# xenji/kafka-topic-analyzer

Measured on AMD Instinct MI355X. Metric: records/sec whole-node + achieved HBM GB/s, 256-part 256B-mean synthetic topic, higher is better.
Workload: dtype u64; 1 GPU; c4: 256-partition synthetic topic, mixed key/value sizes (mean record ~256 B), partitions sharded p % n_gpus; records_per_gpu=1073741824, partitions=256, partition_order=random, bytes_per_record=20, parallelism=partition-sharded x1, forced_collectives=False, exchange=none (1 GPU)

## Files before the change

kafka_topic_analyzer_amd/csrc/kta_api.hip:

```cpp
#include "../../include/kta_hip.h"
#include "kta_compact_delete.h"
#include "kta_compaction.h"
#include "kta_internal.h"
#include "kta_kernels.h"
#include "kta_murmur2.h"
#include "kta_payload.h"
#include "kta_record_batches.h"
#include "kta_segments.h"
#include "kta_size_bins.h"

#include <limits.h>
#include <math.h>
#include <stdio.h>
#include <string.h>

#include <algorithm>
#include <new>
#include <cstdlib>
#include <string>
#include <time.h>
#include <vector>

namespace {

// ... 191 lines not shown

kta_batch *find_allocation(kta_ctx *ctx, const int32_t *p, int32_t *kta_batch::*col, uint64_t *rec0)
{
    const uintptr_t a = reinterpret_cast<uintptr_t>(p);
    for (kta_batch &e : ctx->compact_batches) {
        const uintptr_t lo = reinterpret_cast<uintptr_t>(e.*col);
        if (!p || a < lo || a >= lo + allocation_rows(e) * 4) continue;
        *rec0 = (a - lo) / 4;
        return &e;
    }
    return nullptr;
}

kta_internal_columns columns_at(const kta_internal_columns &rb, uint64_t at)
{
    kta_internal_columns r = rb;
    r.rec0 += at;
    if (!rb.hdr) r.partition += at, r.key_len += at, r.val_len += at, r.ts_ms += at;
    return r;
}
kta::ScanColumns scan_columns(const kta_internal_columns &rb, uint64_t at)
{
    const kta_internal_columns r = columns_at(rb, at);
    return kta::ScanColumns{r.partition, r.key_len, r.val_len, r.ts_ms, r.hdr, r.rec0, r.sum, r.mark};
}
kta::SketchColumns sketch_columns(const kta_internal_columns &rb, const kta_batch *c, uint64_t at)
{
    const kta_internal_columns r = columns_at(rb, at);
    return kta::SketchColumns{r.partition, r.hdr, r.rec0, c->key_len + at, c->key_off + at, c->key_bytes};
}

bool aligned16(const void *p) { return (reinterpret_cast<uintptr_t>(p) & 15u) == 0; }

int widen_lens_for_keys(kta_ctx *ctx, const kta_batch *c, uint64_t n)
{
    uint64_t rec0 = 0;
    const kta_batch *e = find_allocation(ctx, c->key_len, &kta_batch::key_len, &rec0);
    if (!e || e->key_bytes) return KTA_OK;
    const uint64_t rows = allocation_rows(*e), hi = rec0 + n < rows ? rec0 + n : rows;
    KTA_HIP(ctx, kta::launch_tiles_to_raw(e->partition, e->ts_ms, e->key_len, e->val_len, e->tile_hdr, rec0, hi, 2u, true, ctx->s_compute));
    return KTA_OK;
}

constexpr uint64_t kAliveUniqueNum = 2, kAliveUniqueDen = 5;
constexpr int kAliveBackoff = 7;

kta::WrittenList written_list(kta_ctx *ctx) { return kta::WrittenList{ctx->d_written.get(), ctx->d_written_n.get(), ctx->d_written.size()}; }
// ... 1132 lines not shown
    if (!h->partition || !h->key_len || !h->val_len || !h->ts_ms || !d->partition || !d->key_len || !d->val_len || !d->ts_ms)
        return fail(ctx, KTA_ERR_INVALID, "metric columns missing");
    KTA_HIP(ctx, hipSetDevice(ctx->device));
    kta_internal_columns r{};
    int rc = kta_internal_resolve(ctx, d, &r);
    if (rc != KTA_OK) return rc;
    KTA_HIP(ctx, hipStreamSynchronize(ctx->s_compute));
    if (!r.hdr || !r.keyless) {
        KTA_HIP(ctx, hipMemcpy(d->key_len, h->key_len, n * 4, hipMemcpyHostToDevice));
        KTA_HIP(ctx, hipMemcpy(d->val_len, h->val_len, n * 4, hipMemcpyHostToDevice));
    }
    if (!r.hdr) {
        KTA_HIP(ctx, hipMemcpy(d->partition, h->partition, n * 4, hipMemcpyHostToDevice));
        KTA_HIP(ctx, hipMemcpy(d->ts_ms, h->ts_ms, n * 8, hipMemcpyHostToDevice));
        return KTA_OK;
    }
    if (r.rec0 % KTA_TILE_RECORDS)
        return fail(ctx, KTA_ERR_INVALID, "a tile-compact batch is written from a tile boundary");
    const uint64_t nt = tiles_of(n);
    std::vector<int32_t> part(nt * KTA_TILE_RECORDS, 0);
    std::vector<int64_t> ts(nt * KTA_TILE_RECORDS, 0);
    std::vector<kta_tile_hdr> hdr(nt);
    std::vector<kta_tile_sum> sum(nt);
    std::vector<uint32_t> mark(nt, 0u);
    std::vector<int32_t> klen, vlen;
    if (r.keyless) {
        klen.assign(nt * KTA_TILE_RECORDS, 0);
        vlen.assign(nt * KTA_TILE_RECORDS, 0);
    }
    for (uint64_t T = 0; T < nt; T++) {
        const uint64_t a = T * KTA_TILE_RECORDS, m = n - a < KTA_TILE_RECORDS ? n - a : KTA_TILE_RECORDS;
        hdr[T] = kta::tile_pack_host(h->partition + a, h->ts_ms + a, h->key_len + a, h->val_len + a, m, r.keyless, part.data() + a, ts.data() + a,
                                     r.keyless ? klen.data() + a : nullptr, r.keyless ? vlen.data() + a : nullptr, &sum[T]);
        if (r.mark) mark[T] = kta::tile_plane_host(hdr[T], h->partition + a, h->key_len + a, h->val_len + a, m, ts.data() + a);
    }
    if (r.keyless) {
        KTA_HIP(ctx, hipMemcpy(r.key_len + r.rec0, klen.data(), klen.size() * 4, hipMemcpyHostToDevice));
        KTA_HIP(ctx, hipMemcpy(r.val_len + r.rec0, vlen.data(), vlen.size() * 4, hipMemcpyHostToDevice));
    }
    KTA_HIP(ctx, hipMemcpy(r.partition + r.rec0, part.data(), part.size() * 4, hipMemcpyHostToDevice));
    KTA_HIP(ctx, hipMemcpy(r.ts_ms + r.rec0, ts.data(), ts.size() * 8, hipMemcpyHostToDevice));
    KTA_HIP(ctx, hipMemcpy(r.hdr + r.rec0 / KTA_TILE_RECORDS, hdr.data(), nt * sizeof(kta_tile_hdr), hipMemcpyHostToDevice));
    if (r.sum) KTA_HIP(ctx, hipMemcpy(r.sum + r.rec0 / KTA_TILE_RECORDS, sum.data(), nt * sizeof(kta_tile_sum), hipMemcpyHostToDevice));
    if (r.mark) KTA_HIP(ctx, hipMemcpy(r.mark + r.rec0 / KTA_TILE_RECORDS, mark.data(), nt * sizeof(uint32_t), hipMemcpyHostToDevice));
    return KTA_OK;
}

int kta_batch_tile_summaries(kta_ctx *ctx, const kta_batch *d, uint64_t n, kta_tile_sum *out)
{
    if (!ctx || !d || !out) return KTA_ERR_INVALID;
    if (!d->partition) return fail(ctx, KTA_ERR_INVALID, "metric columns missing");
    KTA_HIP(ctx, hipSetDevice(ctx->device));
    kta_internal_columns r{};
    int rc = kta_internal_resolve(ctx, d, &r);
    if (rc != KTA_OK) return rc;
    if (!r.sum) return fail(ctx, KTA_ERR_INVALID, "the batch has no tile summaries (not an allocation of kta_device_batch_alloc)");
    if (r.rec0 % KTA_TILE_RECORDS) return fail(ctx, KTA_ERR_INVALID, "tile summaries are read from a tile boundary");
    if (r.rec0 + n > r.rows) return fail(ctx, KTA_ERR_CAPACITY, "more records than the allocation holds");
    if (n == 0) return KTA_OK;
    KTA_HIP(ctx, hipStreamSynchronize(ctx->s_compute));
    KTA_HIP(ctx, hipMemcpy(out, r.sum + r.rec0 / KTA_TILE_RECORDS, tiles_of(n) * sizeof(kta_tile_sum), hipMemcpyDeviceToHost));
    return KTA_OK;
}

int kta_batch_tile_planes(kta_ctx *ctx, const kta_batch *d, uint64_t n, uint32_t *out)
{
// ... 1276 lines not shown
    const uint64_t base = ctx->next_seq;
    ctx->next_seq += n;
    return base;
}
bool kta_internal_timing(kta_ctx *ctx) { return ctx->timing; }
hipStream_t kta_internal_copy_stream(kta_ctx *ctx) { return ctx->s_copy.get(); }
bool kta_internal_count_alive(kta_ctx *ctx) { return ctx->alive; }
hipStream_t kta_internal_stream(kta_ctx *ctx) { return ctx->s_compute; }
int kta_internal_device(kta_ctx *ctx) { return ctx->device; }
void kta_internal_set_error(kta_ctx *ctx, const char *msg) { ctx->err = msg; }

int kta_internal_prepare_raw(kta_ctx *ctx, const kta_batch *d, uint64_t n)
{
    kta_internal_columns r{};
    int rc = kta_internal_resolve(ctx, d, &r);
    if (rc != KTA_OK || !r.hdr || n == 0) return rc;
    KTA_HIP(ctx, kta::launch_tiles_to_raw(r.partition, r.ts_ms, r.key_len, r.val_len, r.hdr, r.rec0, r.rec0 + n,
                                          r.keyless ? 3u : 1u, false, ctx->s_compute));
    return KTA_OK;
}

int kta_internal_resolve(kta_ctx *ctx, const kta_batch *c, kta_internal_columns *r)
{
    *r = kta_internal_columns{c->partition, c->key_len, c->val_len, c->ts_ms, nullptr, 0, false, 0, nullptr, nullptr};
    uint64_t rec0 = 0;
    if (const kta_batch *e = find_allocation(ctx, c->partition, &kta_batch::partition, &rec0)) {
        if (e->partition + rec0 != c->partition) return fail(ctx, KTA_ERR_INVALID, "a view of a tile-compact batch must start at a record");
        if ((c->ts_ms && c->ts_ms != e->ts_ms + rec0) || (c->key_len && c->key_len != e->key_len + rec0) ||
            (c->val_len && c->val_len != e->val_len + rec0))
            return fail(ctx, KTA_ERR_INVALID, "the columns of a view of a tile-compact batch start at different records");
        *r = kta_internal_columns{e->partition, e->key_len, e->val_len, e->ts_ms, e->tile_hdr, rec0, e->key_bytes == nullptr, allocation_rows(*e),
                                  kta::tile_sums_behind(e->tile_hdr, allocation_rows(*e) / KTA_TILE_RECORDS),
                                  kta::tile_marks_behind(e->tile_hdr, allocation_rows(*e) / KTA_TILE_RECORDS)};
        return KTA_OK;
    }
    if (c->layout == KTA_LAYOUT_TILE_COMPACT) {
        if (!c->tile_hdr) return fail(ctx, KTA_ERR_INVALID, "a tile-compact batch needs its tile headers");
        r->hdr = c->tile_hdr;
    } else if (c->layout != KTA_LAYOUT_RAW) {
        return fail(ctx, KTA_ERR_INVALID, "unknown batch layout");
    }
    return KTA_OK;
}
```

kafka_topic_analyzer_amd/csrc/kta_internal.h:

```cpp
#pragma once

#include <hip/hip_runtime.h>
#include <stddef.h>
#include <stdint.h>

#include <string>
#include <utility>
#include <vector>

#include "kta_hip.h"
#include "kta_kafka.h"

namespace kta {
struct WrittenList;
struct RbFilter;
}

int kta_internal_fail(kta_ctx *ctx, int code, const std::string &msg);
void kta_internal_set_error(kta_ctx *ctx, const char *msg);
void **kta_internal_ext_slot(kta_ctx *ctx, void (*free_fn)(void *));
void **kta_internal_comm_slot(kta_ctx *ctx, void (*free_fn)(void *));
int kta_internal_device(kta_ctx *ctx);
hipStream_t kta_internal_stream(kta_ctx *ctx);
hipStream_t kta_internal_copy_stream(kta_ctx *ctx);
// ... 21 lines not shown
}
struct kta_internal_pl {
    bool on;
    uint64_t *vec;
    int64_t from_ms, to_ms;
    const uint32_t *bitmap;
    int cu_count;
};
bool kta_internal_payload(kta_ctx *ctx, kta_internal_pl *out);
namespace kta {
hipError_t launch_payload(const kta_kafka_batch_desc *descs, uint64_t n, const uint8_t *blob, uint32_t P, int64_t from_ms, int64_t to_ms,
                          const uint32_t *bitmap, uint64_t *vec, int cu_count, uint32_t *workgroups, hipStream_t s);
}
int kta_internal_prepare_raw(kta_ctx *ctx, const kta_batch *d, uint64_t n);
struct kta_internal_columns {
    int32_t *partition, *key_len, *val_len;
    int64_t *ts_ms;
    kta_tile_hdr *hdr;
    uint64_t rec0;
    bool keyless;
    uint64_t rows;
    kta_tile_sum *sum;
    uint32_t *mark;
};
int kta_internal_resolve(kta_ctx *ctx, const kta_batch *d, kta_internal_columns *out);

struct ResultVector {
    uint64_t *out;
    size_t words, sum_words;
    bool max_signed;
};
enum { KTA_RV_COUNTERS = 0, KTA_RV_ANALYTICS, KTA_RV_TIMELINE, KTA_RV_KEY_SKETCH, KTA_RV_HOT_KEYS, KTA_RV_TS_ORDER, KTA_RV_PARTITIONER,
       KTA_RV_SIZE_QUANTILES, KTA_RV_SEGMENTS, KTA_RV_RECORD_BATCHES, KTA_RV_PAYLOAD, KTA_RV_KINDS,
       KTA_SEC_COMPACTION = KTA_RV_KINDS, KTA_SEC_KEPT, KTA_SEC_KINDS };
void kta_internal_result_vectors(kta_ctx *ctx, ResultVector rv[KTA_RV_KINDS]);

static inline int fail(kta_ctx *ctx, int code, const std::string &msg) { return kta_internal_fail(ctx, code, msg); }

static inline int hip_fail(kta_ctx *ctx, hipError_t e, const char *what)
{
    return fail(ctx, e == hipErrorOutOfMemory ? KTA_ERR_NOMEM : KTA_ERR_HIP, std::string(what) + ": " + hipGetErrorString(e));
}

#define KTA_HIP_AS(ctx, call, what)                                \
    do {                                                           \
        hipError_t e__ = (call);                                   \
// ... 132 lines not shown
```

kafka_topic_analyzer_amd/csrc/kta_kernels.h:

```cpp
#pragma once

#include <hip/hip_runtime.h>
#include <stdint.h>

#include "kta_hip.h"
#include "kta_tile.h"
#include "kta_filter.h"

namespace kta {

constexpr int kWG = 256;
constexpr uint32_t kScanCols = 5;
constexpr uint32_t kScanGlobals = 8;
constexpr uint64_t kAliveSlots = 1ull << 32;

enum ScanGlobal : uint32_t {
    SG_TMIN = 0, SG_TMAX = 1, SG_SMIN = 2, SG_SMAX = 3, SG_BAD = 4, SG_NREC = 5
};

struct ScanColumns {
    const int32_t *partition;
    const int32_t *key_len;
    const int32_t *val_len;
    const int64_t *ts_ms;
    const kta_tile_hdr *hdr;
    uint64_t rec0;
    const kta_tile_sum *sum;
    const uint32_t *mark;
};

struct AliveColumns {
    const int32_t *key_len;
    const int32_t *val_len;
    const uint32_t *key_off;
    const uint8_t *key_bytes;
    const uint64_t *seq;
};

struct WrittenList {
    uint32_t *slots;
    unsigned long long *n;
    uint64_t cap;
};

#ifdef __HIPCC__
__device__ __forceinline__ void note_new_slot(const WrittenList &wl, bool is_new, uint32_t slot)
{
    if (!wl.slots) return;
    const unsigned long long m = __ballot(is_new);
    if (m == 0ull) return;
    const uint32_t rank = __builtin_amdgcn_mbcnt_hi((uint32_t)(m >> 32), __builtin_amdgcn_mbcnt_lo((uint32_t)m, 0u));
// ... 246 lines not shown
```

kafka_topic_analyzer_amd/csrc/kta_kernels.hip:

```cpp
#include "kta_kernels.h"

#include <limits.h>
#include <type_traits>

namespace kta {


constexpr uint32_t kCntBits = 21;
constexpr uint64_t kCntMask = (1ull << kCntBits) - 1;
constexpr uint32_t kFlushTiles = 256;
#ifndef KTA_SCAN_PREFETCH
#define KTA_SCAN_PREFETCH 1
#endif
#ifndef KTA_PACKED_LOADS_ONLY
#define KTA_PACKED_LOADS_ONLY 0
#endif
constexpr int kTilePrefetch = KTA_SCAN_PREFETCH;
static_assert(kTilePrefetch == 1 || kTilePrefetch == 2, "the prefetch ring has two or three slots");
#ifndef KTA_PACKED_PREFETCH
#define KTA_PACKED_PREFETCH 1
#endif
constexpr int kPackedPrefetch = KTA_PACKED_PREFETCH;
static_assert(kPackedPrefetch == 1 || kPackedPrefetch == 2, "the prefetch ring has two or three slots");

// ... 584 lines not shown
            uint32_t p = 0; int32_t kl = 0, vl = 0; long long ts = 0;
            if (v) { p = (uint32_t)c.partition[ii]; kl = c.key_len[ii]; vl = c.val_len[ii]; ts = c.ts_ms[ii]; }
            const Rec r = make_rec(p, kl, vl, ts, P, v);
            lane_extrema(r, v, st);
            lds_histograms<ANALYTICS>(r, L);
            lds_record<VARIANT, ANALYTICS>(r, L, rep_log2, rep);
            if (TIMELINE && r.ok) {
                const uint32_t tr = timeline_row(ts, (unsigned long long)ts - (unsigned long long)ta.origin, ta);
                atomicAdd(&T.C[tr], timeline_count(1u, r.tomb));
                atomicAdd(&T.B[tr], (unsigned long long)(r.ks + r.vs));
            }
        }
    }

    flush();
    write_scan_globals(st, s_red, row, P, tid);
}

constexpr uint32_t kFrontFlushTiles = 32;
constexpr uint64_t kFrontRecords = (uint64_t)kFrontFlushTiles * KTA_TILE_RECORDS;
static_assert(kFrontRecords <= 0xFFFFu, "count, tombstones and null keys of a front interval fit 16 bits");
static_assert(kFrontRecords + (kFrontRecords << 16) <= 0xFFFFFFFFull, "count | tombstones << 16 stays in W1's low dword");
static_assert(kFrontRecords * (KTA_COMPACT_LEN_NONE - 1u) < (1ull << 31), "a front interval's u16 sizes sum below 2^31");

struct PackedLds {
    unsigned long long *W1, *W2;
    unsigned long long *B;
};

__device__ __forceinline__ unsigned long long pack_dwords(uint32_t lo, uint32_t hi)
{
    return ((unsigned long long)hi << 32) | lo;
}

template <bool LENS16>
__device__ __forceinline__ void packed_quad_lens(const Quad &q, const uint32_t (&pt)[4], const bool (&ok)[4], uint32_t P,
                                                 uint32_t rep_log2, uint32_t rep, const PackedLds &L, LaneState &st)
{
    uint32_t tomb[4], knull[4], ks[4], vs[4];
    if (LENS16) {
        uint32_t ku[4], vu[4];
        tile_u16x4((uint32_t)q.k.x, (uint32_t)q.k.y, ku);
        tile_u16x4((uint32_t)q.k.z, (uint32_t)q.k.w, vu);
#pragma unroll
        for (int j = 0; j < 4; j++) {
            knull[j] = ku[j] == KTA_COMPACT_LEN_NONE;
// ... 196 lines not shown
#pragma unroll
    for (int j = 0; j < 4; j++) {
        const uint32_t slot = (pt[j] << rep_log2) | rep;
        atomicAdd(&L.W1[slot], pack_dwords(1u | (tomb[j] << 16), ks[j]));
        atomicAdd(&L.W2[slot], pack_dwords(knull[j], vs[j]));
    }
}
__device__ __forceinline__ void lean_quad(const LeanSlot &s, uint32_t rep_log2, uint32_t rep, const PackedLds &L, LaneState &st)
{
    uint32_t pt[4], ku[4], vu[4], tomb[4], knull[4];
    tile_u16x4((uint32_t)s.p.x, (uint32_t)s.p.y, pt);
    tile_u16x4((uint32_t)s.k.x, (uint32_t)s.k.y, ku);
    tile_u16x4((uint32_t)s.k.z, (uint32_t)s.k.w, vu);
#pragma unroll
    for (int j = 0; j < 4; j++) {
        knull[j] = ku[j] == KTA_COMPACT_LEN_NONE;
        tomb[j] = vu[j] == KTA_COMPACT_LEN_NONE;
    }
    lean_quad_add(pt, ku, vu, knull, tomb, rep_log2, rep, L, st);
}
__device__ __forceinline__ void lean_quad(const PlaneSlot &s, uint32_t rep_log2, uint32_t rep, const PackedLds &L, LaneState &st)
{
    const uint32_t w[4] = {(uint32_t)s.w.x, (uint32_t)s.w.y, (uint32_t)s.w.z, (uint32_t)s.w.w};
    uint32_t pt[4], ku[4], vu[4], tomb[4], knull[4];
#pragma unroll
    for (int j = 0; j < 4; j++) {
        pt[j] = w[j] & 0xFFu;
        ku[j] = (w[j] >> 8) & 0xFFu;
        vu[j] = w[j] >> 16;
        knull[j] = ku[j] == KTA_PLANE_KEY_NONE;
        tomb[j] = vu[j] == KTA_COMPACT_LEN_NONE;
    }
    lean_quad_add(pt, ku, vu, knull, tomb, rep_log2, rep, L, st);
}

struct PackedWg {
    PackedLds L;
    uint32_t P, rep_log2, rep, tid;
    LaneState st;

    __device__ __forceinline__ PackedWg(unsigned long long *lds, uint32_t P_, uint32_t rep_log2_) : P(P_), rep_log2(rep_log2_)
    {
        tid = threadIdx.x;
        const uint32_t slots = P << rep_log2;
        L = PackedLds{lds, lds + slots, lds + 2 * slots};
        for (uint32_t i = tid; i < 2 * slots + kScanCols * P; i += kWG) lds[i] = 0ull;
        __syncthreads();
        rep = tid & ((1u << rep_log2) - 1u);
    }
    __device__ __forceinline__ void front_flush() const
    {
        __syncthreads();
        for (uint32_t p = tid; p < P; p += kWG) {
            unsigned long long w1 = 0, w2 = 0;
            for (uint32_t r = 0; r < (1u << rep_log2); r++) {
                const uint32_t s = (p << rep_log2) | r;
                w1 += L.W1[s];
                w2 += L.W2[s];
                L.W1[s] = 0ull;
                L.W2[s] = 0ull;
            }
            L.B[p] += w1 & 0xFFFFull;
            L.B[P + p] += (w1 >> 16) & 0xFFFFull;
            L.B[2u * P + p] += w2 & 0xFFFFFFFFull;
            L.B[3u * P + p] += w1 >> 32;
            L.B[4u * P + p] += w2 >> 32;
        }
        __syncthreads();
    }
    template <bool MERGE = false>
    __device__ __forceinline__ void write_row(uint64_t *row, long long (&s_red)[kWG / 64][6]) const
    {
        for (uint32_t p = tid; p < P; p += kWG)
#pragma unroll
            for (uint32_t j = 0; j < kScanCols; j++) {
                uint64_t &o = row[(uint64_t)p * kScanCols + j];
                if (MERGE) o += L.B[j * P + p];
                else o = L.B[j * P + p];
            }
        write_scan_globals<MERGE>(st, s_red, row, P, tid);
    }
};

constexpr uint32_t kLeanListed = 4;
constexpr uint32_t kScanListA = 5, kScanHandover = 6, kScanListB = 7;
__device__ __forceinline__ uint32_t lean_list_entry(uint64_t list_a, uint64_t list_b, uint32_t i)
{
    return (uint32_t)((i < 2 ? list_a : list_b) >> (32u * (i & 1u)));
}
// ... 41 lines not shown
        if (other) {
            switched = true;
            sw_step = istep;
            stop = issued;
        } else if (in && !v) {
            if (r.listed == kLeanListed) {
                r.handover = istep + 1u;
                r.end = stop = issued;
            } else {
                const uint64_t e = (uint64_t)(istep + 1u) << (32u * (r.listed & 1u));
                if (r.listed < 2) r.list_a |= e;
                else r.list_b |= e;
                r.listed++;
            }
        }
        issued += G;
        istep++;
        look_ahead();
    };
    auto take = [&](const Slot &s, bool v) {
        if (v) {
            lean_quad(s, rep_log2, wg.rep, wg.L, wg.st);
            if (++r.since_flush == kFrontFlushTiles) {
                wg.front_flush();
                r.since_flush = 0;
            }
        }
        r.tile += G;
        r.step++;
    };
    Slot s0, s1, s2, s3;
    bool v0 = false, v1 = false, v2 = false, v3 = false;
    look_ahead();
    issue(s0, v0);
    if (kLeanPrefetch >= 2) issue(s1, v1);
    if (kLeanPrefetch == 3) issue(s2, v2);
    while (r.tile < stop) {
        if (kLeanPrefetch == 3) {
            issue(s3, v3);
            take(s0, v0);
            issue(s0, v0);
            take(s1, v1);
            issue(s1, v1);
            take(s2, v2);
            issue(s2, v2);
            take(s3, v3);
        } else if (kLeanPrefetch == 2) {
            issue(s2, v2);
            take(s0, v0);
            issue(s0, v0);
            take(s1, v1);
            issue(s1, v1);
            take(s2, v2);
        } else {
            issue(s1, v1);
            take(s0, v0);
            issue(s0, v0);
            take(s1, v1);
        }
    }
    if (switched) r.tile = blockIdx.x + sw_step * G, r.step = sw_step;
}

template <bool NT>
__device__ __forceinline__ void packed_scan_lean(const ScanColumns &c, uint64_t n, uint32_t P, uint32_t rep_log2,
                                                 uint64_t *__restrict__ partials, uint32_t row_len, unsigned long long *lds,
                                                 long long (&s_red)[kWG / 64][6])
{
    PackedWg wg(lds, P, rep_log2);
    const uint32_t tid = wg.tid;
    const uint64_t t0 = c.rec0 / KTA_TILE_RECORDS;
    const uint64_t ntiles = (c.rec0 + n + KTA_TILE_RECORDS - 1) / KTA_TILE_RECORDS - t0;
    const uint32_t pc = min(P, (uint32_t)KTA_COMPACT_PART_NONE);
    LeanRun r;
    r.tile = blockIdx.x;
    r.end = (uint32_t)ntiles;
    r.whole_lo = c.rec0 % KTA_TILE_RECORDS ? 1u : 0u;
    r.whole_hi = (uint32_t)((c.rec0 + n) / KTA_TILE_RECORDS - t0);
    const uint32_t last = r.end - 1u;
    bool plane = c.mark != nullptr;
    while (r.tile < r.end) {
        if (plane) lean_run<NT, true>(wg, r, c, t0, last, pc, rep_log2);
        else lean_run<NT, false>(wg, r, c, t0, last, pc, rep_log2);
        plane = !plane;
    }
    for (uint64_t i = blockIdx.x + (uint64_t)tid * gridDim.x; i < r.end; i += (uint64_t)kWG * gridDim.x) {
        const kta_tile_hdr h = c.hdr[t0 + i];
        const kta_tile_sum sm = c.sum[t0 + i];
        const uint32_t mark = c.mark ? c.mark[t0 + i] : 0u;
        bool lean, plane;
        lean_tile(h, sm, mark, i >= r.whole_lo && i < r.whole_hi, pc, lean, plane);
        long long lo, hi;
        tile_sum_extrema(h, sm, lo, hi);
        wg.st.tmin = ((lean || plane) && lo < wg.st.tmin) ? lo : wg.st.tmin;
        wg.st.tmax = ((lean || plane) && hi > wg.st.tmax) ? hi : wg.st.tmax;
    }
    wg.front_flush();
    uint64_t *row = partials + (uint64_t)blockIdx.x * row_len;
    wg.write_row(row, s_red);
    if (tid == 0) {
        uint64_t *g = row + (uint64_t)P * kScanCols;
        g[kScanListA] = r.list_a;
        g[kScanHandover] = r.handover;
        g[kScanListB] = r.list_b;
    }
}

template <bool NT, bool SUM>
__global__ __launch_bounds__(kWG) void kta_metrics_scan_packed(ScanColumns c, uint64_t n, uint32_t P, uint32_t rep_log2,
                                                               uint64_t *__restrict__ partials, uint32_t row_len)
{
    extern __shared__ unsigned long long lds[];
    __shared__ long long s_red[kWG / 64][6];

    if constexpr (SUM) {
        packed_scan_lean<NT>(c, n, P, rep_log2, partials, row_len, lds, s_red);
        return;
    }
    PackedWg wg(lds, P, rep_log2);
    const uint32_t tid = wg.tid;
// ... 279 lines not shown
}

hipError_t launch_metrics_scan(const ScanPlan &pl, const ScanColumns &c, uint64_t n, uint32_t P,
                               uint64_t *partials, hipStream_t s, const TimelineArgs *tl)
{
    if (pl.timeline_rows && (!tl || tl->n_buckets + 3u != pl.timeline_rows)) return hipErrorInvalidValue;
    const bool tiled = c.hdr != nullptr, nt = pl.nontemporal;
    const auto launch = [&](auto kernel, const ScanColumns &cols, const auto &...extra) {
        return launch_scan_kernel(kernel, pl, cols, n, P, partials, s, extra...);
    };
    if (pl.timeline_rows) {
        if (pl.analytics)
            return tiled ? launch(kta_metrics_scan<0, true, true, true, TimelineArgs>, c, *tl)
                         : launch(kta_metrics_scan<0, true, true, false, TimelineArgs>, c, *tl);
        return tiled ? launch(kta_metrics_scan<0, true, false, true, TimelineArgs>, c, *tl)
                     : launch(kta_metrics_scan<0, true, false, false, TimelineArgs>, c, *tl);
    }
    if (pl.analytics) return tiled ? launch(kta_metrics_scan<0, true, true, true>, c) : launch(kta_metrics_scan<0, true, true, false>, c);
    if (pl.packed) {
        if (!tiled) return hipErrorInvalidValue;
        ScanColumns cs = c;
        if (!pl.summaries) cs.sum = nullptr;
        if (!pl.planes || !cs.sum) cs.mark = nullptr;
        if ((c.rec0 % KTA_TILE_RECORDS + n) / KTA_TILE_RECORDS >= (1ull << 31)) cs.sum = nullptr, cs.mark = nullptr;
        if (!cs.sum) return nt ? launch(kta_metrics_scan_packed<true, false>, cs) : launch(kta_metrics_scan_packed<false, false>, cs);
        const hipError_t el = nt ? launch(kta_metrics_scan_packed<true, true>, cs) : launch(kta_metrics_scan_packed<false, true>, cs);
        if (el != hipSuccess) return el;
        return nt ? launch(kta_metrics_scan_packed_rest<true>, cs) : launch(kta_metrics_scan_packed_rest<false>, cs);
    }
    if (pl.variant == 9) {
        if (nt) return tiled ? launch(kta_metrics_scan<9, true, false, true>, c) : launch(kta_metrics_scan<9, true, false, false>, c);
        return tiled ? launch(kta_metrics_scan<9, false, false, true>, c) : launch(kta_metrics_scan<9, false, false, false>, c);
    }
    if (nt) return tiled ? launch(kta_metrics_scan<0, true, false, true>, c) : launch(kta_metrics_scan<0, true, false, false>, c);
    return tiled ? launch(kta_metrics_scan<0, false, false, true>, c) : launch(kta_metrics_scan<0, false, false, false>, c);
}

hipError_t launch_fold_partials(const uint64_t *partials, uint32_t rows, uint32_t P, uint64_t *vec,
                                uint32_t row_len, uint64_t *avec, hipStream_t s)
{
    uint32_t slices = rows < 32 ? rows : 32;
    dim3 grid((row_len + kWG - 1) / kWG, slices), block(kWG);
    hipLaunchKernelGGL(kta_fold_partials, grid, block, 0, s, partials, rows, P, vec, row_len, avec);
    return hipGetLastError();
}

hipError_t launch_tiles_to_raw(int32_t *partition, int64_t *ts_ms, int32_t *key_len, int32_t *val_len, kta_tile_hdr *hdr,
// ... 19 lines not shown
```

kafka_topic_analyzer_amd/csrc/kta_synth.hip:

```cpp
#include "../../include/kta_synth.h"

#include "kta_internal.h"
#include "kta_tile.h"

#include <hip/hip_runtime.h>
#include <limits.h>
#include <string.h>

#include <string>

namespace {

constexpr int kWG = 256;
constexpr int kScanItems = 16;
constexpr int kScanChunk = kWG * kScanItems;

__global__ __launch_bounds__(kWG) void synth_fill_cols(kta_synth_spec sp, uint64_t first, uint64_t n,
                                                       int32_t *part, int32_t *klen, int32_t *vlen,
                                                       int64_t *ts, uint64_t *seq)
{
    const uint64_t stride = (uint64_t)gridDim.x * kWG;
    for (uint64_t i = (uint64_t)blockIdx.x * kWG + threadIdx.x; i < n; i += stride) {
        int32_t p, kl, vl;
        int64_t t;
        kta_synth_record(&sp, first + i, &p, &kl, &vl, &t);
        part[i] = p;
        klen[i] = kl;
        vlen[i] = vl;
        ts[i] = t;
        if (seq) seq[i] = first + i;
    }
}

__global__ __launch_bounds__(kWG) void synth_fill_tiles(kta_synth_spec sp, uint64_t first, uint64_t n, int32_t *part,
                                                        int32_t *klen, int32_t *vlen, int64_t *ts, uint64_t *seq,
                                                        kta_tile_hdr *hdr, kta_tile_sum *sum, uint32_t *mark, uint64_t t0, uint32_t lens16)
{
    __shared__ long long s_red[kWG / 64][4];
    const uint32_t tid = threadIdx.x;
    const uint64_t ntiles = (n + KTA_TILE_RECORDS - 1) / KTA_TILE_RECORDS;
    for (uint64_t T = blockIdx.x; T < ntiles; T += gridDim.x) {
        int32_t p[4], kl[4], vl[4];
        int64_t t[4];
        long long lo = LLONG_MAX, hi = LLONG_MIN, wide = 0;
        long long seen = 0;
        for (uint32_t j = 0; j < 4; j++) {
            const uint64_t i = T * KTA_TILE_RECORDS + 4u * tid + j;
            p[j] = -1;
            t[j] = -1;
            kl[j] = vl[j] = 0;
            if (i >= n) continue;
            kta_synth_record(&sp, first + i, &p[j], &kl[j], &vl[j], &t[j]);
            if (seq) seq[i] = first + i;
            wide |= kta::tile_part_fits(p[j]) ? 0 : 1;
            wide |= kta::tile_len_fits(kl[j]) && kta::tile_len_fits(vl[j]) ? 0 : 2;
            wide |= kta::tile_plane_fits(p[j], kl[j], vl[j]) ? 0 : 4;
            const long long pm = kta::tile_pack_part(p[j]);
            seen = (seen & 0x10000) | ((seen & 0xFFFF) > pm ? (seen & 0xFFFF) : pm) | (t[j] == -1 ? 0x10000 : 0);
            if (t[j] != -1) {
                lo = t[j] < lo ? t[j] : lo;
                hi = t[j] > hi ? t[j] : hi;
            }
        }
        for (int off = 32; off > 0; off >>= 1) {
            const long long a = __shfl_xor(lo, off), b = __shfl_xor(hi, off), c = __shfl_xor(wide, off), d = __shfl_xor(seen, off);
            lo = a < lo ? a : lo;
            hi = b > hi ? b : hi;
            wide |= c;
            seen = ((seen | d) & 0x10000) | ((seen & 0xFFFF) > (d & 0xFFFF) ? (seen & 0xFFFF) : (d & 0xFFFF));
        }
        if ((tid & 63u) == 0u) {
            s_red[tid >> 6][0] = lo;
            s_red[tid >> 6][1] = hi;
            s_red[tid >> 6][2] = wide;
            s_red[tid >> 6][3] = seen;
        }
        __syncthreads();
        for (uint32_t w = 0; w < kWG / 64; w++) {
            lo = s_red[w][0] < lo ? s_red[w][0] : lo;
            hi = s_red[w][1] > hi ? s_red[w][1] : hi;
            wide |= s_red[w][2];
            const long long d = s_red[w][3];
            seen = ((seen | d) & 0x10000) | ((seen & 0xFFFF) > (d & 0xFFFF) ? (seen & 0xFFFF) : (d & 0xFFFF));
        }
        __syncthreads();
        int64_t base;
        const bool compact = kta::tile_ts_fits(lo, hi, &base) && !(wide & 1);
        const uint64_t A = (t0 + T) * KTA_TILE_RECORDS;
        if (compact) {
            uint16_t u[4];
            int32_t o[4];
            for (uint32_t j = 0; j < 4; j++) {
                u[j] = kta::tile_pack_part(p[j]);
                o[j] = kta::tile_pack_ts(t[j], base);
            }
            reinterpret_cast<uint2 *>(part)[(2 * A) / 4 + tid] =
                make_uint2(kta::tile_u16x2_word(u[0], u[1]), kta::tile_u16x2_word(u[2], u[3]));
            reinterpret_cast<int4 *>(ts)[(2 * A) / 4 + tid] = make_int4(o[0], o[1], o[2], o[3]);
        } else {
            reinterpret_cast<int4 *>(part)[A / 4 + tid] = make_int4(p[0], p[1], p[2], p[3]);
            reinterpret_cast<longlong2 *>(ts)[A / 2 + 2 * tid] = make_longlong2(t[0], t[1]);
            reinterpret_cast<longlong2 *>(ts)[A / 2 + 2 * tid + 1] = make_longlong2(t[2], t[3]);
        }
        const bool u16 = lens16 && !(wide & 2);
        if (u16) {
            using kta::tile_pack_len;
            reinterpret_cast<uint4 *>(klen)[A / 4 + tid] =
                make_uint4(kta::tile_u16x2_word(tile_pack_len(kl[0]), tile_pack_len(kl[1])), kta::tile_u16x2_word(tile_pack_len(kl[2]), tile_pack_len(kl[3])),
                           kta::tile_u16x2_word(tile_pack_len(vl[0]), tile_pack_len(vl[1])), kta::tile_u16x2_word(tile_pack_len(vl[2]), tile_pack_len(vl[3])));
        } else {
            reinterpret_cast<int4 *>(klen)[A / 4 + tid] = make_int4(kl[0], kl[1], kl[2], kl[3]);
            reinterpret_cast<int4 *>(vlen)[A / 4 + tid] = make_int4(vl[0], vl[1], vl[2], vl[3]);
        }
        const bool plane = mark && compact && !(wide & 4) && n - T * KTA_TILE_RECORDS >= KTA_TILE_RECORDS;
        if (plane)
            reinterpret_cast<uint4 *>(ts)[A / 2 + kta::kTilePlaneOffset / 16u + tid] =
                make_uint4(kta::tile_plane_pack(p[0], kl[0], vl[0]), kta::tile_plane_pack(p[1], kl[1], vl[1]),
                           kta::tile_plane_pack(p[2], kl[2], vl[2]), kta::tile_plane_pack(p[3], kl[3], vl[3]));
        if (tid == 0) {
            if (mark) mark[t0 + T] = plane ? 1u : 0u;
            hdr[t0 + T] = kta_tile_hdr{compact ? base : 0, compact ? KTA_TILE_COMPACT : KTA_TILE_RAW, u16 ? KTA_TILE_LENS_U16 : KTA_TILE_LENS_I32};
            const uint64_t m = n - T * KTA_TILE_RECORDS < KTA_TILE_RECORDS ? n - T * KTA_TILE_RECORDS : KTA_TILE_RECORDS;
            if (sum) sum[t0 + T] = compact ? kta::tile_summary(lo, hi, (uint32_t)(seen & 0xFFFF), (seen & 0x10000) != 0, m) : kta_tile_sum{0, 0, 0};
        }
    }
}

__device__ __forceinline__ uint32_t klen_bytes(const int32_t *klen, uint64_t i, uint64_t n)
{
    if (i >= n) return 0u;
    const int32_t k = klen[i];
    return k > 0 ? (uint32_t)k : 0u;
}

__global__ __launch_bounds__(kWG) void synth_chunk_sums(const int32_t *klen, uint64_t n, uint64_t *chunk_sum)
{
    __shared__ uint64_t s[kWG];
    const uint64_t base = (uint64_t)blockIdx.x * kScanChunk + (uint64_t)threadIdx.x * kScanItems;
    uint64_t t = 0;
    for (int j = 0; j < kScanItems; j++) t += klen_bytes(klen, base + j, n);
    s[threadIdx.x] = t;
    __syncthreads();
// ... 132 lines not shown
int kta_synth_fill_device(kta_ctx *ctx, const kta_synth_spec *spec, uint64_t first, uint64_t n,
                          const kta_batch *b, uint64_t *n_key_bytes)
{
    if (!ctx || !b) return KTA_ERR_INVALID;
    if (check_spec(spec) != KTA_OK) return fail(ctx, KTA_ERR_INVALID, "invalid synthetic spec");
    if (n > b->capacity) return fail(ctx, KTA_ERR_CAPACITY, "synthetic batch larger than the device batch capacity");
    if (n_key_bytes) *n_key_bytes = 0;
    if (n == 0) return KTA_OK;
    hipStream_t s = kta_internal_stream(ctx);
    KTA_HIP(ctx, hipSetDevice(kta_internal_device(ctx)));
    const uint32_t grid = (uint32_t)((n + kWG - 1) / kWG < 8192 ? (n + kWG - 1) / kWG : 8192);
    kta_internal_columns ac{};
    if (int rc = kta_internal_resolve(ctx, b, &ac)) return rc;
    kta_tile_hdr *ahdr = ac.hdr;
    const uint64_t rec0 = ac.rec0;
    if (ahdr && rec0 % KTA_TILE_RECORDS != 0) {
        if (int rc = kta_internal_prepare_raw(ctx, b, n)) return rc;
        ahdr = nullptr;
    }
    if (ahdr) {
        const uint64_t nt = (n + KTA_TILE_RECORDS - 1) / KTA_TILE_RECORDS;
        const uint32_t lens16 = ac.keyless && !b->key_off && !b->key_bytes ? 1u : 0u;
        hipLaunchKernelGGL(synth_fill_tiles, dim3((uint32_t)(nt < 8192 ? nt : 8192)), dim3(kWG), 0, s, *spec, first, n, ac.partition,
                           ac.key_len, ac.val_len, ac.ts_ms, b->seq, ahdr, ac.sum, ac.mark, rec0 / KTA_TILE_RECORDS, lens16);
    } else {
        hipLaunchKernelGGL(synth_fill_cols, dim3(grid), dim3(kWG), 0, s, *spec, first, n, b->partition, b->key_len,
                           b->val_len, b->ts_ms, b->seq);
    }
    KTA_HIP(ctx, hipGetLastError());
    uint64_t total = 0;
    if (b->key_off && b->key_bytes) {
        const uint64_t n_chunks = (n + kScanChunk - 1) / kScanChunk;
        DeviceBuf<uint64_t> chunks;
        if (hipError_t e = chunks.alloc(n_chunks + 1))
            return fail(ctx, KTA_ERR_HIP, std::string("chunks.alloc(n_chunks + 1): ") + hipGetErrorString(e));
        uint64_t *const d_chunks = chunks.get();
        hipLaunchKernelGGL(synth_chunk_sums, dim3((uint32_t)n_chunks), dim3(kWG), 0, s, b->key_len, n, d_chunks);
        hipLaunchKernelGGL(synth_scan_chunks, dim3(1), dim3(1024), 0, s, d_chunks, n_chunks, d_chunks + n_chunks);
        KTA_HIP(ctx, hipGetLastError());
        KTA_HIP(ctx, hipMemcpyAsync(&total, d_chunks + n_chunks, sizeof(uint64_t), hipMemcpyDeviceToHost, s));
        KTA_HIP(ctx, hipStreamSynchronize(s));
        if (total > b->key_bytes_capacity || total >= (1ull << 32)) {
            if (n_key_bytes) *n_key_bytes = total;
            return fail(ctx, KTA_ERR_CAPACITY, "synthetic key bytes exceed the device batch key capacity");
        }
        hipLaunchKernelGGL(synth_key_offsets, dim3((uint32_t)n_chunks), dim3(kWG), 0, s, b->key_len, n, d_chunks,
                           b->key_off);
// ... 70 lines not shown
```

kafka_topic_analyzer_amd/csrc/kta_tile.h:

```cpp
#pragma once

#include <stdint.h>
#include <string.h>

#include "kta_hip.h"

#ifdef __HIPCC__
#define KTA_TILE_HD __host__ __device__
#else
#define KTA_TILE_HD
#endif

namespace kta {

KTA_TILE_HD inline bool tile_part_fits(int32_t p) { return p >= -1 && p < (int32_t)KTA_COMPACT_PART_NONE; }
KTA_TILE_HD inline bool tile_len_fits(int32_t l) { return l >= -1 && l < (int32_t)KTA_COMPACT_LEN_NONE; }
KTA_TILE_HD inline bool tile_ts_fits(int64_t lo, int64_t hi, int64_t *base)
{
    *base = lo <= hi ? lo : 0;
    return lo > hi || (uint64_t)hi - (uint64_t)lo <= (uint64_t)INT32_MAX;
}

KTA_TILE_HD inline kta_tile_sum *tile_sums_behind(kta_tile_hdr *hdr, uint64_t ntiles)
{
    return reinterpret_cast<kta_tile_sum *>(hdr + ntiles);
}
static_assert(sizeof(kta_tile_sum) == 8 && sizeof(kta_tile_hdr) == 16, "a summary is one 8-byte word behind 16-byte headers");
KTA_TILE_HD inline kta_tile_sum tile_summary(int64_t lo, int64_t hi, uint32_t part_max, bool untimed, uint64_t m)
{
    kta_tile_sum s{0, 0, 0};
    if (m != KTA_TILE_RECORDS) return s;
    const bool timed = lo <= hi;
    s.ts_span = timed ? (uint32_t)((uint64_t)hi - (uint64_t)lo) : 0u;
    s.part_max = (uint16_t)part_max;
    s.flags = (uint16_t)(KTA_TILE_SUM_VALID | (timed ? KTA_TILE_SUM_TIMED : 0u) | (untimed ? KTA_TILE_SUM_UNTIMED : 0u));
    return s;
}

constexpr uint32_t KTA_PLANE_PARTS = 256u, KTA_PLANE_KEY_NONE = 0xFFu;
constexpr uint32_t kTilePlaneOffset = KTA_TILE_RECORDS * 4u;
KTA_TILE_HD inline uint32_t *tile_marks_behind(kta_tile_hdr *hdr, uint64_t ntiles)
{
    return reinterpret_cast<uint32_t *>(tile_sums_behind(hdr, ntiles) + ntiles);
}
constexpr uint64_t kTileSideBytes = sizeof(kta_tile_hdr) + sizeof(kta_tile_sum) + sizeof(uint32_t);
KTA_TILE_HD inline bool tile_plane_fits(int32_t p, int32_t k, int32_t v)
{
    return p >= 0 && p < (int32_t)KTA_PLANE_PARTS && k >= -1 && k < (int32_t)KTA_PLANE_KEY_NONE && tile_len_fits(v);
}
KTA_TILE_HD inline uint32_t tile_plane_pack(int32_t p, int32_t k, int32_t v)
{
    return (uint32_t)p | (((uint32_t)k & 0xFFu) << 8) | ((uint32_t)v << 16);
}
KTA_TILE_HD inline int32_t tile_plane_part(uint32_t w) { return (int32_t)(w & 0xFFu); }
KTA_TILE_HD inline int32_t tile_plane_key(uint32_t w) { return ((w >> 8) & 0xFFu) == KTA_PLANE_KEY_NONE ? -1 : (int32_t)((w >> 8) & 0xFFu); }
KTA_TILE_HD inline int32_t tile_plane_val(uint32_t w) { return (w >> 16) == KTA_COMPACT_LEN_NONE ? -1 : (int32_t)(w >> 16); }
KTA_TILE_HD inline uint32_t tile_plane_at(uint32_t j) { return kTilePlaneOffset + 4u * j; }

KTA_TILE_HD inline uint16_t tile_pack_part(int32_t p) { return p == -1 ? (uint16_t)KTA_COMPACT_PART_NONE : (uint16_t)p; }
KTA_TILE_HD inline int32_t tile_unpack_part(uint32_t u) { return u == KTA_COMPACT_PART_NONE ? -1 : (int32_t)u; }
KTA_TILE_HD inline int32_t tile_pack_ts(int64_t t, int64_t base)
{
    return t == -1 ? KTA_COMPACT_TS_NONE : (int32_t)((uint64_t)t - (uint64_t)base);
}
KTA_TILE_HD inline int64_t tile_unpack_ts(int32_t o, int64_t base)
{
    return o == KTA_COMPACT_TS_NONE ? -1 : (int64_t)((uint64_t)base + (uint64_t)(int64_t)o);
}
// ... 57 lines not shown
    } else {
        memcpy(klen, k, m * 4);
        memcpy(vlen, v, m * 4);
    }
    return h;
}

inline void tile_unpack_host(const kta_tile_hdr &h, const int32_t *part, const int64_t *ts, const int32_t *klen, const int32_t *vlen,
                             uint64_t j0, uint64_t j1, int32_t *p, int64_t *t, int32_t *k, int32_t *v)
{
    const uint16_t *p16 = reinterpret_cast<const uint16_t *>(part), *g16 = reinterpret_cast<const uint16_t *>(klen);
    const int32_t *o32 = reinterpret_cast<const int32_t *>(ts);
    for (uint64_t j = j0; j < j1; j++) {
        const bool compact = h.mode == KTA_TILE_COMPACT;
        p[j - j0] = compact ? tile_unpack_part(p16[tile_compact_at(j, 0)]) : part[j];
        t[j - j0] = compact ? tile_unpack_ts(o32[tile_compact_at(j, 0)], h.ts_base) : ts[j];
        if (!klen) continue;
        const bool u16 = h.lens == KTA_TILE_LENS_U16;
        k[j - j0] = u16 ? tile_unpack_len(g16[tile_klen_slot((uint32_t)j)]) : klen[j];
        v[j - j0] = u16 ? tile_unpack_len(g16[tile_vlen_slot((uint32_t)j)]) : vlen[j];
    }
}

inline uint32_t tile_plane_host(const kta_tile_hdr &h, const int32_t *p, const int32_t *k, const int32_t *v, uint64_t m, int64_t *ts)
{
    if (h.mode != KTA_TILE_COMPACT || m != KTA_TILE_RECORDS) return 0u;
    for (uint64_t j = 0; j < m; j++)
        if (!tile_plane_fits(p[j], k[j], v[j])) return 0u;
    unsigned char *plane = reinterpret_cast<unsigned char *>(ts);
    for (uint64_t j = 0; j < m; j++) {
        const uint32_t w = tile_plane_pack(p[j], k[j], v[j]);
        memcpy(plane + tile_plane_at((uint32_t)j), &w, 4);
    }
    return 1u;
}

#ifdef __HIPCC__
template <bool NT, bool TS = true>
__device__ __forceinline__ void tile_record_h(const int32_t *part, const int64_t *ts, const kta_tile_hdr &h, uint64_t tile,
                                              uint64_t i, int32_t &p, long long &t)
{
    if (h.mode == KTA_TILE_COMPACT) {
        const uint64_t ci = tile_compact_at(i, tile);
        const uint16_t *p16 = reinterpret_cast<const uint16_t *>(part) + ci;
        p = tile_unpack_part(NT ? __builtin_nontemporal_load(p16) : *p16);
        if (TS) {
            const int32_t *t32 = reinterpret_cast<const int32_t *>(ts) + ci;
            t = tile_unpack_ts(NT ? __builtin_nontemporal_load(t32) : *t32, h.ts_base);
        }
    } else {
        p = NT ? __builtin_nontemporal_load(part + i) : part[i];
        if (TS) t = NT ? __builtin_nontemporal_load(ts + i) : ts[i];
    }
}

template <bool NT, bool TS = true>
// ... 43 lines not shown
```

Before: 1184 billion records/s.

## Precompute per-tile size extrema and simplify plane quad accumulation with raw sentinel correction

Adds a per-tile min/max record-size side array, filled at write time by the synth kernel and the host tile packer. The scan reads these extrema instead of deriving them per record. The plane-path lean_quad now adds raw key and value lengths with sentinel values included, plus a fast path of one atomic pair when all four records share a partition. The front flush subtracts the sentinel contributions afterwards. This moves per-record decode work into a side table and fewer LDS atomics, at the cost of extra side bytes per tile and a flush after each run.

```diff
diff --git a/kafka_topic_analyzer_amd/csrc/kta_api.hip b/kafka_topic_analyzer_amd/csrc/kta_api.hip
--- a/kafka_topic_analyzer_amd/csrc/kta_api.hip
+++ b/kafka_topic_analyzer_amd/csrc/kta_api.hip
@@ -237,7 +237,7 @@
 kta::ScanColumns scan_columns(const kta_internal_columns &rb, uint64_t at)
 {
     const kta_internal_columns r = columns_at(rb, at);
-    return kta::ScanColumns{r.partition, r.key_len, r.val_len, r.ts_ms, r.hdr, r.rec0, r.sum, r.mark};
+    return kta::ScanColumns{r.partition, r.key_len, r.val_len, r.ts_ms, r.hdr, r.rec0, r.sum, r.mark, r.size};
 }
 kta::SketchColumns sketch_columns(const kta_internal_columns &rb, const kta_batch *c, uint64_t at)
 {
@@ -1416,7 +1416,7 @@
     std::vector<int64_t> ts(nt * KTA_TILE_RECORDS, 0);
     std::vector<kta_tile_hdr> hdr(nt);
     std::vector<kta_tile_sum> sum(nt);
-    std::vector<uint32_t> mark(nt, 0u);
+    std::vector<uint32_t> mark(nt, 0u), size(2 * nt, 0u);
     std::vector<int32_t> klen, vlen;
     if (r.keyless) {
         klen.assign(nt * KTA_TILE_RECORDS, 0);
@@ -1426,7 +1426,7 @@
         const uint64_t a = T * KTA_TILE_RECORDS, m = n - a < KTA_TILE_RECORDS ? n - a : KTA_TILE_RECORDS;
         hdr[T] = kta::tile_pack_host(h->partition + a, h->ts_ms + a, h->key_len + a, h->val_len + a, m, r.keyless, part.data() + a, ts.data() + a,
                                      r.keyless ? klen.data() + a : nullptr, r.keyless ? vlen.data() + a : nullptr, &sum[T]);
-        if (r.mark) mark[T] = kta::tile_plane_host(hdr[T], h->partition + a, h->key_len + a, h->val_len + a, m, ts.data() + a);
+        if (r.mark) mark[T] = kta::tile_plane_host(hdr[T], h->partition + a, h->key_len + a, h->val_len + a, m, ts.data() + a, &size[2 * T]);
     }
     if (r.keyless) {
         KTA_HIP(ctx, hipMemcpy(r.key_len + r.rec0, klen.data(), klen.size() * 4, hipMemcpyHostToDevice));
@@ -1436,6 +1436,7 @@
     KTA_HIP(ctx, hipMemcpy(r.ts_ms + r.rec0, ts.data(), ts.size() * 8, hipMemcpyHostToDevice));
     KTA_HIP(ctx, hipMemcpy(r.hdr + r.rec0 / KTA_TILE_RECORDS, hdr.data(), nt * sizeof(kta_tile_hdr), hipMemcpyHostToDevice));
     if (r.sum) KTA_HIP(ctx, hipMemcpy(r.sum + r.rec0 / KTA_TILE_RECORDS, sum.data(), nt * sizeof(kta_tile_sum), hipMemcpyHostToDevice));
+    if (r.mark) KTA_HIP(ctx, hipMemcpy(r.size + 2 * (r.rec0 / KTA_TILE_RECORDS), size.data(), 2 * nt * sizeof(uint32_t), hipMemcpyHostToDevice));
     if (r.mark) KTA_HIP(ctx, hipMemcpy(r.mark + r.rec0 / KTA_TILE_RECORDS, mark.data(), nt * sizeof(uint32_t), hipMemcpyHostToDevice));
     return KTA_OK;
 }
@@ -2758,7 +2759,7 @@
 
 int kta_internal_resolve(kta_ctx *ctx, const kta_batch *c, kta_internal_columns *r)
 {
-    *r = kta_internal_columns{c->partition, c->key_len, c->val_len, c->ts_ms, nullptr, 0, false, 0, nullptr, nullptr};
+    *r = kta_internal_columns{c->partition, c->key_len, c->val_len, c->ts_ms, nullptr, 0, false, 0, nullptr, nullptr, nullptr};
     uint64_t rec0 = 0;
     if (const kta_batch *e = find_allocation(ctx, c->partition, &kta_batch::partition, &rec0)) {
         if (e->partition + rec0 != c->partition) return fail(ctx, KTA_ERR_INVALID, "a view of a tile-compact batch must start at a record");
@@ -2767,7 +2768,8 @@
             return fail(ctx, KTA_ERR_INVALID, "the columns of a view of a tile-compact batch start at different records");
         *r = kta_internal_columns{e->partition, e->key_len, e->val_len, e->ts_ms, e->tile_hdr, rec0, e->key_bytes == nullptr, allocation_rows(*e),
                                   kta::tile_sums_behind(e->tile_hdr, allocation_rows(*e) / KTA_TILE_RECORDS),
-                                  kta::tile_marks_behind(e->tile_hdr, allocation_rows(*e) / KTA_TILE_RECORDS)};
+                                  kta::tile_marks_behind(e->tile_hdr, allocation_rows(*e) / KTA_TILE_RECORDS),
+                                  kta::tile_sizes_behind(e->tile_hdr, allocation_rows(*e) / KTA_TILE_RECORDS)};
         return KTA_OK;
     }
     if (c->layout == KTA_LAYOUT_TILE_COMPACT) {
diff --git a/kafka_topic_analyzer_amd/csrc/kta_internal.h b/kafka_topic_analyzer_amd/csrc/kta_internal.h
--- a/kafka_topic_analyzer_amd/csrc/kta_internal.h
+++ b/kafka_topic_analyzer_amd/csrc/kta_internal.h
@@ -67,6 +67,7 @@
     uint64_t rows;
     kta_tile_sum *sum;
     uint32_t *mark;
+    uint32_t *size;
 };
 int kta_internal_resolve(kta_ctx *ctx, const kta_batch *d, kta_internal_columns *out);
 
diff --git a/kafka_topic_analyzer_amd/csrc/kta_kernels.h b/kafka_topic_analyzer_amd/csrc/kta_kernels.h
--- a/kafka_topic_analyzer_amd/csrc/kta_kernels.h
+++ b/kafka_topic_analyzer_amd/csrc/kta_kernels.h
@@ -27,6 +27,7 @@
     uint64_t rec0;
     const kta_tile_sum *sum;
     const uint32_t *mark;
+    const uint32_t *size;
 };
 
 struct AliveColumns {
diff --git a/kafka_topic_analyzer_amd/csrc/kta_kernels.hip b/kafka_topic_analyzer_amd/csrc/kta_kernels.hip
--- a/kafka_topic_analyzer_amd/csrc/kta_kernels.hip
+++ b/kafka_topic_analyzer_amd/csrc/kta_kernels.hip
@@ -630,6 +630,8 @@
 static_assert(kFrontRecords <= 0xFFFFu, "count, tombstones and null keys of a front interval fit 16 bits");
 static_assert(kFrontRecords + (kFrontRecords << 16) <= 0xFFFFFFFFull, "count | tombstones << 16 stays in W1's low dword");
 static_assert(kFrontRecords * (KTA_COMPACT_LEN_NONE - 1u) < (1ull << 31), "a front interval's u16 sizes sum below 2^31");
+static_assert(kFrontRecords * KTA_PLANE_KEY_NONE < (1ull << 23), "a front interval's raw plane key bytes sum below 2^23");
+static_assert(kFrontRecords * KTA_COMPACT_LEN_NONE < (1ull << 31), "a front interval's raw plane value words sum below 2^31");
 
 struct PackedLds {
     unsigned long long *W1, *W2;
@@ -872,6 +874,10 @@
 __device__ __forceinline__ void lean_quad(const PlaneSlot &s, uint32_t rep_log2, uint32_t rep, const PackedLds &L, LaneState &st)
 {
     const uint32_t w[4] = {(uint32_t)s.w.x, (uint32_t)s.w.y, (uint32_t)s.w.z, (uint32_t)s.w.w};
+#if KTA_PACKED_LOADS_ONLY
+    st.bad += w[0] ^ w[1] ^ w[2] ^ w[3];
+    return;
+#endif
     uint32_t pt[4], ku[4], vu[4], tomb[4], knull[4];
 #pragma unroll
     for (int j = 0; j < 4; j++) {
@@ -881,7 +887,20 @@
         knull[j] = ku[j] == KTA_PLANE_KEY_NONE;
         tomb[j] = vu[j] == KTA_COMPACT_LEN_NONE;
     }
-    lean_quad_add(pt, ku, vu, knull, tomb, rep_log2, rep, L, st);
+    if (pt[0] == pt[1] && pt[0] == pt[2] && pt[0] == pt[3]) {
+        const uint32_t slot = (pt[0] << rep_log2) | rep;
+        const uint32_t tombs = tomb[0] + tomb[1] + tomb[2] + tomb[3];
+        const uint32_t knulls = knull[0] + knull[1] + knull[2] + knull[3];
+        atomicAdd(&L.W1[slot], pack_dwords(4u | (tombs << 16), ku[0] + ku[1] + ku[2] + ku[3]));
+        atomicAdd(&L.W2[slot], pack_dwords(knulls, vu[0] + vu[1] + vu[2] + vu[3]));
+        return;
+    }
+#pragma unroll
+    for (int j = 0; j < 4; j++) {
+        const uint32_t slot = (pt[j] << rep_log2) | rep;
+        atomicAdd(&L.W1[slot], pack_dwords(1u | (tomb[j] << 16), ku[j]));
+        atomicAdd(&L.W2[slot], pack_dwords(knull[j], vu[j]));
+    }
 }
 
 struct PackedWg {
@@ -898,8 +917,9 @@
         __syncthreads();
         rep = tid & ((1u << rep_log2) - 1u);
     }
-    __device__ __forceinline__ void front_flush() const
+    __device__ __forceinline__ void front_flush(bool raw = false) const
     {
+        const unsigned long long key_none = raw ? KTA_PLANE_KEY_NONE : 0u, val_none = raw ? KTA_COMPACT_LEN_NONE : 0u;
         __syncthreads();
         for (uint32_t p = tid; p < P; p += kWG) {
             unsigned long long w1 = 0, w2 = 0;
@@ -913,8 +933,8 @@
             L.B[p] += w1 & 0xFFFFull;
             L.B[P + p] += (w1 >> 16) & 0xFFFFull;
             L.B[2u * P + p] += w2 & 0xFFFFFFFFull;
-            L.B[3u * P + p] += w1 >> 32;
-            L.B[4u * P + p] += w2 >> 32;
+            L.B[3u * P + p] += (w1 >> 32) - key_none * (w2 & 0xFFFFFFFFull);
+            L.B[4u * P + p] += (w2 >> 32) - val_none * ((w1 >> 16) & 0xFFFFull);
         }
         __syncthreads();
     }
@@ -1002,12 +1022,11 @@
         if (v) {
             lean_quad(s, rep_log2, wg.rep, wg.L, wg.st);
             if (++r.since_flush == kFrontFlushTiles) {
-                wg.front_flush();
+                wg.front_flush(PLANE);
                 r.since_flush = 0;
             }
         }
         r.tile += G;
-        r.step++;
     };
     Slot s0, s1, s2, s3;
     bool v0 = false, v1 = false, v2 = false, v3 = false;
@@ -1039,6 +1058,7 @@
             take(s1, v1);
         }
     }
+    r.step = istep - (uint32_t)kLeanPrefetch;
     if (switched) r.tile = blockIdx.x + sw_step * G, r.step = sw_step;
 }
 
@@ -1062,6 +1082,10 @@
     while (r.tile < r.end) {
         if (plane) lean_run<NT, true>(wg, r, c, t0, last, pc, rep_log2);
         else lean_run<NT, false>(wg, r, c, t0, last, pc, rep_log2);
+        if (r.since_flush) {
+            wg.front_flush(plane);
+            r.since_flush = 0;
+        }
         plane = !plane;
     }
     for (uint64_t i = blockIdx.x + (uint64_t)tid * gridDim.x; i < r.end; i += (uint64_t)kWG * gridDim.x) {
@@ -1074,8 +1098,11 @@
         tile_sum_extrema(h, sm, lo, hi);
         wg.st.tmin = ((lean || plane) && lo < wg.st.tmin) ? lo : wg.st.tmin;
         wg.st.tmax = ((lean || plane) && hi > wg.st.tmax) ? hi : wg.st.tmax;
-    }
-    wg.front_flush();
+        if (plane) {
+            wg.st.smin = min(wg.st.smin, c.size[2 * (t0 + i)]);
+            wg.st.smax = max(wg.st.smax, c.size[2 * (t0 + i) + 1]);
+        }
+    }
     uint64_t *row = partials + (uint64_t)blockIdx.x * row_len;
     wg.write_row(row, s_red);
     if (tid == 0) {
@@ -1401,7 +1428,8 @@
         ScanColumns cs = c;
         if (!pl.summaries) cs.sum = nullptr;
         if (!pl.planes || !cs.sum) cs.mark = nullptr;
-        if ((c.rec0 % KTA_TILE_RECORDS + n) / KTA_TILE_RECORDS >= (1ull << 31)) cs.sum = nullptr, cs.mark = nullptr;
+        if (!cs.mark) cs.size = nullptr;
+        if ((c.rec0 % KTA_TILE_RECORDS + n) / KTA_TILE_RECORDS >= (1ull << 31)) cs.sum = nullptr, cs.mark = nullptr, cs.size = nullptr;
         if (!cs.sum) return nt ? launch(kta_metrics_scan_packed<true, false>, cs) : launch(kta_metrics_scan_packed<false, false>, cs);
         const hipError_t el = nt ? launch(kta_metrics_scan_packed<true, true>, cs) : launch(kta_metrics_scan_packed<false, true>, cs);
         if (el != hipSuccess) return el;
diff --git a/kafka_topic_analyzer_amd/csrc/kta_synth.hip b/kafka_topic_analyzer_amd/csrc/kta_synth.hip
--- a/kafka_topic_analyzer_amd/csrc/kta_synth.hip
+++ b/kafka_topic_analyzer_amd/csrc/kta_synth.hip
@@ -34,9 +34,9 @@
 
 __global__ __launch_bounds__(kWG) void synth_fill_tiles(kta_synth_spec sp, uint64_t first, uint64_t n, int32_t *part,
                                                         int32_t *klen, int32_t *vlen, int64_t *ts, uint64_t *seq,
-                                                        kta_tile_hdr *hdr, kta_tile_sum *sum, uint32_t *mark, uint64_t t0, uint32_t lens16)
-{
-    __shared__ long long s_red[kWG / 64][4];
+                                                        kta_tile_hdr *hdr, kta_tile_sum *sum, uint32_t *mark, uint32_t *size, uint64_t t0, uint32_t lens16)
+{
+    __shared__ long long s_red[kWG / 64][5];
     const uint32_t tid = threadIdx.x;
     const uint64_t ntiles = (n + KTA_TILE_RECORDS - 1) / KTA_TILE_RECORDS;
     for (uint64_t T = blockIdx.x; T < ntiles; T += gridDim.x) {
@@ -44,6 +44,7 @@
         int64_t t[4];
         long long lo = LLONG_MAX, hi = LLONG_MIN, wide = 0;
         long long seen = 0;
+        uint32_t slo = kta::kTileSizeMinNone, shi = kta::kTileSizeMaxNone;
         for (uint32_t j = 0; j < 4; j++) {
             const uint64_t i = T * KTA_TILE_RECORDS + 4u * tid + j;
             p[j] = -1;
@@ -55,6 +56,7 @@
             wide |= kta::tile_part_fits(p[j]) ? 0 : 1;
             wide |= kta::tile_len_fits(kl[j]) && kta::tile_len_fits(vl[j]) ? 0 : 2;
             wide |= kta::tile_plane_fits(p[j], kl[j], vl[j]) ? 0 : 4;
+            kta::tile_size_fold(kl[j], vl[j], slo, shi);
             const long long pm = kta::tile_pack_part(p[j]);
             seen = (seen & 0x10000) | ((seen & 0xFFFF) > pm ? (seen & 0xFFFF) : pm) | (t[j] == -1 ? 0x10000 : 0);
             if (t[j] != -1) {
@@ -68,12 +70,15 @@
             hi = b > hi ? b : hi;
             wide |= c;
             seen = ((seen | d) & 0x10000) | ((seen & 0xFFFF) > (d & 0xFFFF) ? (seen & 0xFFFF) : (d & 0xFFFF));
+            slo = min(slo, (uint32_t)__shfl_xor((int)slo, off));
+            shi = max(shi, (uint32_t)__shfl_xor((int)shi, off));
         }
         if ((tid & 63u) == 0u) {
             s_red[tid >> 6][0] = lo;
             s_red[tid >> 6][1] = hi;
             s_red[tid >> 6][2] = wide;
             s_red[tid >> 6][3] = seen;
+            s_red[tid >> 6][4] = (long long)(((unsigned long long)slo << 32) | shi);
         }
         __syncthreads();
         for (uint32_t w = 0; w < kWG / 64; w++) {
@@ -82,6 +87,9 @@
             wide |= s_red[w][2];
             const long long d = s_red[w][3];
             seen = ((seen | d) & 0x10000) | ((seen & 0xFFFF) > (d & 0xFFFF) ? (seen & 0xFFFF) : (d & 0xFFFF));
+            const unsigned long long e = (unsigned long long)s_red[w][4];
+            slo = min(slo, (uint32_t)(e >> 32));
+            shi = max(shi, (uint32_t)e);
         }
         __syncthreads();
         int64_t base;
@@ -118,6 +126,7 @@
                 make_uint4(kta::tile_plane_pack(p[0], kl[0], vl[0]), kta::tile_plane_pack(p[1], kl[1], vl[1]),
                            kta::tile_plane_pack(p[2], kl[2], vl[2]), kta::tile_plane_pack(p[3], kl[3], vl[3]));
         if (tid == 0) {
+            if (plane) size[2 * (t0 + T)] = slo, size[2 * (t0 + T) + 1] = shi;
             if (mark) mark[t0 + T] = plane ? 1u : 0u;
             hdr[t0 + T] = kta_tile_hdr{compact ? base : 0, compact ? KTA_TILE_COMPACT : KTA_TILE_RAW, u16 ? KTA_TILE_LENS_U16 : KTA_TILE_LENS_I32};
             const uint64_t m = n - T * KTA_TILE_RECORDS < KTA_TILE_RECORDS ? n - T * KTA_TILE_RECORDS : KTA_TILE_RECORDS;
@@ -296,7 +305,7 @@
         const uint64_t nt = (n + KTA_TILE_RECORDS - 1) / KTA_TILE_RECORDS;
         const uint32_t lens16 = ac.keyless && !b->key_off && !b->key_bytes ? 1u : 0u;
         hipLaunchKernelGGL(synth_fill_tiles, dim3((uint32_t)(nt < 8192 ? nt : 8192)), dim3(kWG), 0, s, *spec, first, n, ac.partition,
-                           ac.key_len, ac.val_len, ac.ts_ms, b->seq, ahdr, ac.sum, ac.mark, rec0 / KTA_TILE_RECORDS, lens16);
+                           ac.key_len, ac.val_len, ac.ts_ms, b->seq, ahdr, ac.sum, ac.mark, ac.size, rec0 / KTA_TILE_RECORDS, lens16);
     } else {
         hipLaunchKernelGGL(synth_fill_cols, dim3(grid), dim3(kWG), 0, s, *spec, first, n, b->partition, b->key_len,
                            b->val_len, b->ts_ms, b->seq);
diff --git a/kafka_topic_analyzer_amd/csrc/kta_tile.h b/kafka_topic_analyzer_amd/csrc/kta_tile.h
--- a/kafka_topic_analyzer_amd/csrc/kta_tile.h
+++ b/kafka_topic_analyzer_amd/csrc/kta_tile.h
@@ -43,7 +43,19 @@
 {
     return reinterpret_cast<uint32_t *>(tile_sums_behind(hdr, ntiles) + ntiles);
 }
-constexpr uint64_t kTileSideBytes = sizeof(kta_tile_hdr) + sizeof(kta_tile_sum) + sizeof(uint32_t);
+constexpr uint32_t kTileSizeMinNone = 0xFFFFFFFFu, kTileSizeMaxNone = 0u;
+KTA_TILE_HD inline uint32_t *tile_sizes_behind(kta_tile_hdr *hdr, uint64_t ntiles)
+{
+    return tile_marks_behind(hdr, ntiles) + ntiles;
+}
+constexpr uint64_t kTileSideBytes = sizeof(kta_tile_hdr) + sizeof(kta_tile_sum) + sizeof(uint32_t) + 2 * sizeof(uint32_t);
+KTA_TILE_HD inline void tile_size_fold(int32_t k, int32_t v, uint32_t &lo, uint32_t &hi)
+{
+    if (v == -1) return;
+    const uint32_t sz = (uint32_t)(k == -1 ? 0 : k) + (uint32_t)v;
+    lo = sz < lo ? sz : lo;
+    hi = sz > hi ? sz : hi;
+}
 KTA_TILE_HD inline bool tile_plane_fits(int32_t p, int32_t k, int32_t v)
 {
     return p >= 0 && p < (int32_t)KTA_PLANE_PARTS && k >= -1 && k < (int32_t)KTA_PLANE_KEY_NONE && tile_len_fits(v);
@@ -147,16 +159,20 @@
     }
 }
 
-inline uint32_t tile_plane_host(const kta_tile_hdr &h, const int32_t *p, const int32_t *k, const int32_t *v, uint64_t m, int64_t *ts)
+inline uint32_t tile_plane_host(const kta_tile_hdr &h, const int32_t *p, const int32_t *k, const int32_t *v, uint64_t m, int64_t *ts,
+                                uint32_t *sizes = nullptr)
 {
     if (h.mode != KTA_TILE_COMPACT || m != KTA_TILE_RECORDS) return 0u;
     for (uint64_t j = 0; j < m; j++)
         if (!tile_plane_fits(p[j], k[j], v[j])) return 0u;
     unsigned char *plane = reinterpret_cast<unsigned char *>(ts);
+    uint32_t lo = kTileSizeMinNone, hi = kTileSizeMaxNone;
     for (uint64_t j = 0; j < m; j++) {
         const uint32_t w = tile_plane_pack(p[j], k[j], v[j]);
         memcpy(plane + tile_plane_at((uint32_t)j), &w, 4);
-    }
+        tile_size_fold(k[j], v[j], lo, hi);
+    }
+    if (sizes) sizes[0] = lo, sizes[1] = hi;
     return 1u;
 }
 
```

Measured after the change: 1241 billion records/s, median of 6. 4.8% higher.
